# beecave-homelab/VibeVoice-ROCm

Measured on AMD Instinct MI355X. Metric: audio-sec/s, higher is better.
Workload: dtype bf16

## Files before the change

### vibevoice_rocm_amd/csrc/vv_common.h

```cpp
#ifndef VV_COMMON_H
#define VV_COMMON_H
#include <hip/hip_runtime.h>
#include <stdarg.h>
#include <stdint.h>
#include "vv_hip.h"

int vv_set_error(int code, const char* fmt, ...);

#define VV_CHECK_LAUNCH(name)                                                                    \
  do {                                                                                           \
    hipError_t e_ = hipGetLastError();                                                           \
    if (e_ != hipSuccess) return vv_set_error(VV_E_HIP, "%s: %s", name, hipGetErrorString(e_));  \
  } while (0)

#define VV_TRY(expr)            \
  do {                          \
    int rc_ = (expr);           \
    if (rc_) return rc_;        \
  } while (0)

int vv_launch_gemv_stream(const vv_lin_args& a, hipStream_t s);
int vv_launch_gemv_rows(const vv_lin_args& a, float* part, size_t part_floats, int* tickets, size_t n_tickets, hipStream_t s);
size_t vv_gemv_rows_part_floats(int n, int dual);
size_t vv_gemv_rows_tickets(int n);
int vv_gemv_rows_init();
void vv_gemv_rows_set(int on, int blocks, int pers);
int vv_linear_ws(const vv_lin_args* a, const void* f1, const void* f2, float* part, size_t part_floats, int* tickets, size_t n_tickets,
                 vv_stream_t stream, const vv_w8* q1 = nullptr, const vv_w8* q2 = nullptr);
int vv_launch_mfma_gemm(const vv_lin_args& a, hipStream_t s);
int vv_mfma_gemm_init();
int vv_launch_attn_decode(const float* qkv, int64_t ld_qkv, int R, int heads, const vv_kv* kv, int layer, const float2* rope, const int* lens, float* out,
                          int64_t ldo, float* part, int* tickets, int nsplit, int part_cap, hipStream_t s);
int vv_attn_decode_ws(const float* qkv, int64_t ld_qkv, int R, int heads, const vv_kv* kv, int layer, const float* rope_table, const int* lens, float* out,
                      int64_t ldo, float* part, int* tickets, int nsplit, int part_cap, vv_stream_t stream);
int vv_launch_attn_prefill(const float* qkv, int64_t ld_qkv, int R, int heads, const vv_kv* kv, int layer, const int* lens, const int* cache_rows,
                           float* out, int64_t ldo, hipStream_t s);
int vv_head_init_fused(const vv_head* h, const float* noise, float* Xs, float* Ms, float* h0, int64_t ldh, hipStream_t s);
bool vv_head_boundary_supported(const vv_head* h);
int vv_head_boundary_fused(const vv_head* h, const float* hrows, int64_t ldh, const float* shift, const float* scale, int64_t ld_mod, float cfg,
                           const vv_dpm_coef* k, float* Xs, float* Ms, float* h_out, int64_t ldh_out, float* latent_out, hipStream_t s);
int vv_head_boundary_batch(const vv_head* h, const float* hrows, int64_t ldh, const float* shift, const float* scale, int64_t ld_mod, float cfg,
                           const vv_dpm_coef* k, float* Xs, float* Ms, int64_t state_stride, float* h_out, int64_t ldh_out, float* latent_out,
                           int64_t latent_stride, int B, hipStream_t s,
                           const float* nx = nullptr, int64_t nx_stride = 0);
int vv_head_sde_proj_fused(const vv_head* h, const float* sde_noise, int64_t ld_sde, int n_steps, int B, float* NX, hipStream_t s);
int vv_fused_init();
int vv_head_pre_fused(const vv_head* h, const float* cond2, int64_t ld_cond, const float* temb, int n_steps, void* c_bf16, const float* noise,
                      float* Xs, float* Ms, float* h0, int64_t ldh, hipStream_t s);
int vv_launch_connector_pair(const vv_connector* ac, const vv_connector* sem, const float* latent, const float* semfeat, float* out, int64_t ldo, int rows_out,
                             float* ws, hipStream_t s);
int vv_head_modulations_fused(const vv_head* h, const void* c_bf16, int rows, float* const* mod, float* modf, hipStream_t s);
struct vv_conv_ctx_item { float* pad; float* state; int ctx, T, C; const float* dw_w; float* hs; int affine; float scale, bias; };
int vv_conv_ctx_batch(const vv_conv_ctx_item* items, int n, int scatter, hipStream_t s);
int vv_block1d_init();
int vv_launch_block1d(const vv_block& B, int wdt, const float* x, float* out, int T, int C, float eps, hipStream_t s);
void vv_block1d_set_fused(int on);
void vv_block1d_set_blocks(int b);
int vv_convffn_init();
int vv_launch_convffn(const vv_block& B, int wdt, const float* x, float* y, void* hidden, float* hist_new, float* out, int T, int C, float eps,
                      hipStream_t s);
void vv_convffn_set(int on);
int vv_launch_ffn_in_row(const vv_block& B, int wdt, const float* x, float* y, float* hidden, float* hist_new, int C, float eps, hipStream_t s);
void vv_convffn_set_t1(int on);
int vv_launch_ffn_in_row_hs(const vv_block& B, int wdt, const float* x, float* y, float* hidden, float* hist_new, int C, float eps, hipStream_t s);
void vv_convffn_set_t1hs(int on);
void vv_convffn_set_rows(int c, int rows);
void vv_convffn_set_c128(int on);
bool vv_convffn_prefers(int wdt, int T, int C);
int vv_launch_skinny(const vv_lin_args& a, hipStream_t s);
void vv_skinny_set(int on, int min_m, int max_m);
int vv_rmsnorm_rows(const float* x, int64_t ldx, const float* w, float eps, int rows, int n, float* out, int64_t ldo, hipStream_t s);

#ifdef __HIPCC__
__device__ __forceinline__ float vv_gelu_as(float v) {
  const float x = v * 0.70710678118654752440f, ax = fabsf(x);
  const float t = __builtin_amdgcn_rcpf(fmaf(0.3275911f, ax, 1.0f));
  const float poly = t * fmaf(t, fmaf(t, fmaf(t, fmaf(t, 1.061405429f, -1.453152027f), 1.421413741f), -0.284496736f), 0.254829592f);
  const float erf_abs = 1.0f - poly * __expf(-ax * ax);
  return 0.5f * v * (1.0f + copysignf(erf_abs, x));
}

__device__ __forceinline__ float vv_wave_sum(float v) {
#define VV_DPP_ADD(ctrl) v += __int_as_float(__builtin_amdgcn_update_dpp(0, __float_as_int(v), ctrl, 0xF, 0xF, true))
  VV_DPP_ADD(0xB1);
  VV_DPP_ADD(0x4E);
  VV_DPP_ADD(0x141);
  VV_DPP_ADD(0x140);
#undef VV_DPP_ADD
  const float r0 = __int_as_float(__builtin_amdgcn_readlane(__float_as_int(v), 0));
  const float r1 = __int_as_float(__builtin_amdgcn_readlane(__float_as_int(v), 16));
  const float r2 = __int_as_float(__builtin_amdgcn_readlane(__float_as_int(v), 32));
  const float r3 = __int_as_float(__builtin_amdgcn_readlane(__float_as_int(v), 48));
  return (r0 + r1) + (r2 + r3);
}
#endif

#endif
```

### vibevoice_rocm_amd/csrc/vv_convffn.hip

```cpp
#include <hip/hip_runtime.h>
#include <hip/hip_bf16.h>
#include <stdint.h>

#include "vv_hip.h"
#include "vv_common.h"

namespace {

typedef unsigned short bf16_t;
typedef __bf16 bf16x8 __attribute__((ext_vector_type(8)));
typedef float f32x16 __attribute__((ext_vector_type(16)));
typedef float f32x4 __attribute__((ext_vector_type(4)));
typedef unsigned int u32x4 __attribute__((ext_vector_type(4)));

#ifdef VV_CF_TIMING
__device__ unsigned long long g_cf_t[8];
#define CSTAMP(i) do { if (blockIdx.x == 0 && blockIdx.y == 0 && threadIdx.x == 0) { const long long t_ = wall_clock64(); g_cf_t[i] += (unsigned long long)(t_ - tprev_); tprev_ = t_; } } while (0)
#else
#define CSTAMP(i) do { } while (0)
#endif

constexpr int TR2 = 16;
constexpr int HALO = 6;

__device__ __forceinline__ unsigned int pack2(float a, float b) {
  const __hip_bfloat16 x = __float2bfloat16(a), y = __float2bfloat16(b);
  return (unsigned int)(*reinterpret_cast<const bf16_t*>(&x)) | ((unsigned int)(*reinterpret_cast<const bf16_t*>(&y)) << 16);
}
__device__ __forceinline__ float sq4(const float4 v) { return v.x * v.x + v.y * v.y + v.z * v.z + v.w * v.w; }

template <int C, int TRV, int NT = 256> struct InLay {
  static constexpr int VW = C >= 256 ? 4 : 2;
  static constexpr int F4 = C / 4;
  static constexpr int FV = C / VW;
  static constexpr int TPR = FV < NT ? FV : NT;
  static constexpr int NWV = NT / 64;
  static constexpr int CPT = FV / TPR;
  static constexpr int RP = NT / TPR;
  static constexpr int NI = (TRV + HALO + RP - 1) / RP;
  static constexpr int WR = NI * RP;
  static constexpr int WPR = TPR / 64;
  static constexpr int P1 = C + 8;
  static constexpr int ST = C / (16 * NWV);
  static constexpr size_t XN = (size_t)WR * C * 4;
  static constexpr size_t RED = (size_t)NWV * 16 * 64 * 4;
  static constexpr size_t XH = (size_t)(WR - HALO) * P1 * 2;
  static constexpr size_t PART = (size_t)2 * WR * 8 * 4;
  static constexpr size_t LDS = (XN > RED ? XN : RED) + XH + PART;
};

template <int VW> __device__ __forceinline__ void ldv(const float* p, float (&o)[VW]) {
  if constexpr (VW == 4) { const float4 t = *reinterpret_cast<const float4*>(p); o[0] = t.x; o[1] = t.y; o[2] = t.z; o[3] = t.w; }
  else { const float2 t = *reinterpret_cast<const float2*>(p); o[0] = t.x; o[1] = t.y; }
}
template <int VW> __device__ __forceinline__ void stv(float* p, const float (&o)[VW]) {
  if constexpr (VW == 4) *reinterpret_cast<float4*>(p) = make_float4(o[0], o[1], o[2], o[3]);
  else *reinterpret_cast<float2*>(p) = make_float2(o[0], o[1]);
}

template <int C, int TRV, bool HF32, int NT>
__global__ __launch_bounds__(NT) void ffn_in_kernel(const float* __restrict__ x, float* __restrict__ y, void* __restrict__ hidden_v,
                                                     float* __restrict__ hist_new, int T, const vv_block B, float eps) {
  using L = InLay<C, TRV, NT>;
  constexpr int TR = TRV, CPT = L::CPT, VW = L::VW, NWV = L::NWV;
#ifdef VV_CF_TIMING
  long long tprev_ = wall_clock64();
#endif
  extern __shared__ __attribute__((aligned(16))) unsigned char smem[];
  float* xn = reinterpret_cast<float*>(smem);
  float* red = reinterpret_cast<float*>(smem);
  bf16_t* xh = reinterpret_cast<bf16_t*>(smem + (L::XN > L::RED ? L::XN : L::RED));
  float* part = reinterpret_cast<float*>(smem + (L::XN > L::RED ? L::XN : L::RED) + L::XH);
  float* part2 = part + L::WR * 8;
  const int tid = threadIdx.x, lane = tid & 63, wave = __builtin_amdgcn_readfirstlane(tid >> 6);
  const int n0 = blockIdx.x * 32;
  const int t0 = blockIdx.y * TR;
  const int rows = min(TR, T - t0);
  const int lm = lane & 31, hk = (lane >> 5) * 8;

  const int rloc = wave / L::WPR, slot = wave % L::WPR;
  int c0[CPT];
#pragma unroll
  for (int j = 0; j < CPT; ++j) c0[j] = VW * (tid % L::TPR + L::TPR * j);
  const float* hb = B.hist ? B.hist : x;
  const float hkeep = B.hist ? 1.f : 0.f;
  float own[L::NI][CPT][VW];
#pragma unroll
  for (int i = 0; i < L::NI; ++i) {
    const int w = rloc + L::RP * i, t = t0 - HALO + w;
    const bool isx = t >= 0;
    const float* src = isx ? x + (int64_t)min(t, T - 1) * C : hb + (int64_t)(B.hist ? HALO + t : 0) * C;
    const float keep = (w < rows + HALO) ? (isx ? 1.f : hkeep) : 0.f;
#pragma unroll
    for (int j = 0; j < CPT; ++j) {
      ldv<VW>(src + c0[j], own[i][j]);
#pragma unroll
      for (int e = 0; e < VW; ++e) own[i][j][e] *= keep;
    }
  }
  float nw[CPT][VW], db[CPT][VW], gm[CPT][VW], fw[CPT][VW];
  float tap[CPT][VW * 7];
#pragma unroll
  for (int j = 0; j < CPT; ++j) {
    ldv<VW>(B.norm_w + c0[j], nw[j]);
    ldv<VW>(B.dw_b + c0[j], db[j]);
    ldv<VW>(B.gamma + c0[j], gm[j]);
    ldv<VW>(B.ffn_norm_w + c0[j], fw[j]);
#pragma unroll
    for (int q = 0; q < 7; ++q) {
      float tq[VW];
      ldv<VW>(B.dw_w + (size_t)c0[j] * 7 + VW * q, tq);
#pragma unroll
      for (int e = 0; e < VW; ++e) tap[j][VW * q + e] = tq[e];
    }
  }
  u32x4 wf[L::ST];
  {
    const bf16_t* wr = reinterpret_cast<const bf16_t*>(B.w1) + (int64_t)(n0 + lm) * C + wave * (C / NWV) + hk;
#pragma unroll
    for (int s = 0; s < L::ST; ++s) wf[s] = *reinterpret_cast<const u32x4*>(wr + s * 16);
  }
  const int eg = wave & 3;
  const float4 b1v = *reinterpret_cast<const float4*>(B.b1 + n0 + 8 * eg + 4 * (lane >> 5));
  __builtin_amdgcn_sched_barrier(0);

  CSTAMP(0);
#pragma unroll
  for (int i = 0; i < L::NI; ++i) {
    const int w = rloc + L::RP * i;
    float q = 0.f;
#pragma unroll
    for (int j = 0; j < CPT; ++j)
#pragma unroll
      for (int e = 0; e < VW; ++e) q = fmaf(own[i][j][e], own[i][j][e], q);
    const float s = vv_wave_sum(q);
    if (lane == 0) part[w * 8 + slot] = s;
  }
  __syncthreads();
  CSTAMP(1);
#pragma unroll
  for (int i = 0; i < L::NI; ++i) {
    const int w = rloc + L::RP * i, t = t0 - HALO + w;
    float ss = part[w * 8];
#pragma unroll
    for (int sl = 1; sl < L::WPR; ++sl) ss += part[w * 8 + sl];
    const bool isx = t >= 0;
    const float rstd = isx ? rsqrtf(ss / (float)C + eps) : 1.f;
#pragma unroll
    for (int j = 0; j < CPT; ++j) {
      float o[VW];
#pragma unroll
      for (int e = 0; e < VW; ++e) o[e] = own[i][j][e] * rstd * (isx ? nw[j][e] : 1.f);
      stv<VW>(xn + w * C + c0[j], o);
    }
  }
  __syncthreads();
  CSTAMP(2);

  float y1[L::NI][CPT][VW];
#pragma unroll
  for (int i = 0; i < L::NI; ++i) {
#pragma unroll
    for (int j = 0; j < CPT; ++j)
#pragma unroll
      for (int e = 0; e < VW; ++e) y1[i][j][e] = 0.f;
    if (L::RP * i + L::RP - 1 < HALO) continue;
    const int w = rloc + L::RP * i, tt = w - HALO;
    const int tc = max(tt, 0);
    const float ok = (tt >= 0 && tt < rows) ? 1.f : 0.f;
    float q = 0.f;
#pragma unroll
    for (int j = 0; j < CPT; ++j) {
      float s[VW];
#pragma unroll
      for (int e = 0; e < VW; ++e) s[e] = db[j][e];
#pragma unroll
      for (int k = 0; k < 7; ++k) {
        float v[VW];
        ldv<VW>(xn + (tc + k) * C + c0[j], v);
#pragma unroll
        for (int e = 0; e < VW; ++e) s[e] = fmaf(tap[j][7 * e + k], v[e], s[e]);
      }
#pragma unroll
      for (int e = 0; e < VW; ++e) {
        y1[i][j][e] = (own[i][j][e] + gm[j][e] * s[e]) * ok;
        q = fmaf(y1[i][j][e], y1[i][j][e], q);
      }
    }
    const float s2 = vv_wave_sum(q);
    if (lane == 0) part2[w * 8 + slot] = s2;
  }
  if (hist_new && blockIdx.x == 0 && t0 + TR >= T) {
    for (int e = tid; e < HALO * L::F4; e += NT) {
      const int j = e / L::F4, c4 = e - j * L::F4;
      *reinterpret_cast<float4*>(hist_new + (size_t)j * C + 4 * c4) = *reinterpret_cast<const float4*>(xn + (size_t)(T - t0 + j) * C + 4 * c4);
    }
  }
  __syncthreads();
  CSTAMP(3);
  {
    const int ys0 = blockIdx.x * (C / (int)gridDim.x);
#pragma unroll
    for (int i = 0; i < L::NI; ++i) {
      if (L::RP * i + L::RP - 1 < HALO) continue;
      const int w = rloc + L::RP * i, tt = w - HALO;
      if (tt >= 0) {
        float ss = part2[w * 8];
#pragma unroll
        for (int sl = 1; sl < L::WPR; ++sl) ss += part2[w * 8 + sl];
        const float rstd = rsqrtf(ss / (float)C + eps);
#pragma unroll
        for (int j = 0; j < CPT; ++j) {
          if constexpr (VW == 4) {
            uint2 p;
            p.x = pack2(y1[i][j][0] * rstd * fw[j][0], y1[i][j][1] * rstd * fw[j][1]);
            p.y = pack2(y1[i][j][2] * rstd * fw[j][2], y1[i][j][3] * rstd * fw[j][3]);
            *reinterpret_cast<uint2*>(xh + tt * L::P1 + c0[j]) = p;
          } else {
            *reinterpret_cast<unsigned int*>(xh + tt * L::P1 + c0[j]) = pack2(y1[i][j][0] * rstd * fw[j][0], y1[i][j][1] * rstd * fw[j][1]);
          }
          const bool mine = c0[j] >= ys0 && c0[j] < ys0 + C / (int)gridDim.x;
          if (mine && tt < rows) stv<VW>(y + (int64_t)(t0 + tt) * C + c0[j], y1[i][j]);
        }
      }
    }
  }
  __syncthreads();

  CSTAMP(4);
  f32x16 acc;
#pragma unroll
  for (int i = 0; i < 16; ++i) acc[i] = 0.f;
  {
    const bf16_t* xf = xh + min(lm, TR - 1) * L::P1 + wave * (C / NWV) + hk;
#pragma unroll
    for (int s = 0; s < L::ST; ++s) {
      const u32x4 xb = *reinterpret_cast<const u32x4*>(xf + s * 16);
      acc = __builtin_amdgcn_mfma_f32_32x32x16_bf16(__builtin_bit_cast(bf16x8, wf[s]), __builtin_bit_cast(bf16x8, xb), acc, 0, 0, 0);
    }
  }
#pragma unroll
  for (int r = 0; r < 16; ++r) red[(wave * 16 + r) * 64 + lane] = acc[r];
  __syncthreads();
  CSTAMP(5);
  {
    const int m = lane & 31;
    if (m < rows && wave < 4) {
      float v[4];
#pragma unroll
      for (int i = 0; i < 4; ++i) {
        float s = 0.f;
#pragma unroll
        for (int w4 = 0; w4 < NWV; ++w4) s += red[(w4 * 16 + 4 * eg + i) * 64 + lane];
        v[i] = s;
      }
      const float g0 = vv_gelu_as(v[0] + b1v.x), g1 = vv_gelu_as(v[1] + b1v.y), g2 = vv_gelu_as(v[2] + b1v.z), g3 = vv_gelu_as(v[3] + b1v.w);
      const int64_t ho = (int64_t)(t0 + m) * (4 * C) + n0 + 8 * eg + 4 * (lane >> 5);
      if (HF32) {
        *reinterpret_cast<float4*>(reinterpret_cast<float*>(hidden_v) + ho) = make_float4(g0, g1, g2, g3);
      } else {
        uint2 p;
        p.x = pack2(g0, g1);
        p.y = pack2(g2, g3);
        *reinterpret_cast<uint2*>(reinterpret_cast<bf16_t*>(hidden_v) + ho) = p;
      }
    }
  }
  CSTAMP(6);
}


__global__ __launch_bounds__(256) void ffn_in_row_kernel(const float* __restrict__ x, float* __restrict__ y, float* __restrict__ hidden,
                                                         float* __restrict__ hist_new, const vv_block B, float eps) {
  constexpr int C = 2048, P1 = C + 8, ST = C / 64;
  __shared__ __attribute__((aligned(16))) bf16_t xh[P1];
  __shared__ float red[4 * 16 * 64];
  __shared__ float part[8];
  const int tid = threadIdx.x, lane = tid & 63, wave = __builtin_amdgcn_readfirstlane(tid >> 6);
  const int n0 = blockIdx.x * 32;
  const int lm = lane & 31, hk = (lane >> 5) * 8;
  float xv[2][4], hsv[2][4], dl[2][4], nw[2][4], db[2][4], gm[2][4], fw[2][4];
  int c0[2];
#pragma unroll
  for (int j = 0; j < 2; ++j) {
    c0[j] = 4 * (tid + 256 * j);
    ldv<4>(x + c0[j], xv[j]);
    ldv<4>(B.norm_w + c0[j], nw[j]);
    ldv<4>(B.hs + c0[j], hsv[j]);
    ldv<4>(B.dw_last + c0[j], dl[j]);
    ldv<4>(B.dw_b + c0[j], db[j]);
    ldv<4>(B.gamma + c0[j], gm[j]);
    ldv<4>(B.ffn_norm_w + c0[j], fw[j]);
  }
  const bool keeper = hist_new && blockIdx.x == 0;
  float hrow[5][2][4];
  if (keeper) {
#pragma unroll
    for (int r = 0; r < 5; ++r)
#pragma unroll
      for (int j = 0; j < 2; ++j) ldv<4>(B.hist + (size_t)(r + 1) * C + c0[j], hrow[r][j]);
  }
  u32x4 wf[ST];
  {
    const bf16_t* wr = reinterpret_cast<const bf16_t*>(B.w1) + (int64_t)(n0 + lm) * C + wave * (C / 4) + hk;
#pragma unroll
    for (int s = 0; s < ST; ++s) wf[s] = *reinterpret_cast<const u32x4*>(wr + s * 16);
  }
  const int eg = wave;
  const float4 b1v = *reinterpret_cast<const float4*>(B.b1 + n0 + 8 * eg + 4 * (lane >> 5));
  __builtin_amdgcn_sched_barrier(0);
  float q = 0.f;
#pragma unroll
  for (int j = 0; j < 2; ++j)
#pragma unroll
    for (int e = 0; e < 4; ++e) q = fmaf(xv[j][e], xv[j][e], q);
  q = vv_wave_sum(q);
  if (lane == 0) part[wave] = q;
  __syncthreads();
  const float rstd1 = rsqrtf(((part[0] + part[1]) + (part[2] + part[3])) / (float)C + eps);
  float yv[2][4], xn[2][4];
  float q2 = 0.f;
#pragma unroll
  for (int j = 0; j < 2; ++j)
#pragma unroll
    for (int e = 0; e < 4; ++e) {
      xn[j][e] = xv[j][e] * rstd1 * nw[j][e];
      const float sc = db[j][e] + hsv[j][e] + dl[j][e] * xn[j][e];
      yv[j][e] = xv[j][e] + gm[j][e] * sc;
      q2 = fmaf(yv[j][e], yv[j][e], q2);
    }
  q2 = vv_wave_sum(q2);
  if (lane == 0) part[4 + wave] = q2;
  if (keeper) {
#pragma unroll
    for (int j = 0; j < 2; ++j) {
#pragma unroll
      for (int r = 0; r < 5; ++r) stv<4>(hist_new + (size_t)r * C + c0[j], hrow[r][j]);
      stv<4>(hist_new + (size_t)5 * C + c0[j], xn[j]);
    }
  }
  __syncthreads();
  const float rstd2 = rsqrtf(((part[4] + part[5]) + (part[6] + part[7])) / (float)C + eps);
  {
    const int ys0 = blockIdx.x * (C / (int)gridDim.x);
#pragma unroll
    for (int j = 0; j < 2; ++j) {
      uint2 p;
      p.x = pack2(yv[j][0] * rstd2 * fw[j][0], yv[j][1] * rstd2 * fw[j][1]);
      p.y = pack2(yv[j][2] * rstd2 * fw[j][2], yv[j][3] * rstd2 * fw[j][3]);
      *reinterpret_cast<uint2*>(xh + c0[j]) = p;
      if (c0[j] >= ys0 && c0[j] < ys0 + C / (int)gridDim.x) stv<4>(y + c0[j], yv[j]);
    }
  }
  __syncthreads();
  f32x16 acc;
#pragma unroll
  for (int i = 0; i < 16; ++i) acc[i] = 0.f;
  {
    const bf16_t* xf = xh + wave * (C / 4) + hk;
#pragma unroll
    for (int s = 0; s < ST; ++s) {
      const u32x4 xb = *reinterpret_cast<const u32x4*>(xf + s * 16);
      acc = __builtin_amdgcn_mfma_f32_32x32x16_bf16(__builtin_bit_cast(bf16x8, wf[s]), __builtin_bit_cast(bf16x8, xb), acc, 0, 0, 0);
    }
  }
#pragma unroll
  for (int r = 0; r < 16; ++r) red[(wave * 16 + r) * 64 + lane] = acc[r];
  __syncthreads();
  if ((lane & 31) == 0) {
    float v[4];
#pragma unroll
    for (int i = 0; i < 4; ++i) {
      float s = 0.f;
#pragma unroll
      for (int w4 = 0; w4 < 4; ++w4) s += red[(w4 * 16 + 4 * eg + i) * 64 + lane];
      v[i] = s;
    }
    *reinterpret_cast<float4*>(hidden + n0 + 8 * eg + 4 * (lane >> 5)) =
        make_float4(vv_gelu_as(v[0] + b1v.x), vv_gelu_as(v[1] + b1v.y), vv_gelu_as(v[2] + b1v.z), vv_gelu_as(v[3] + b1v.w));
  }
}

template <int C, int NW>
__global__ __launch_bounds__(64 * NW) void ffn_out_kernel(const bf16_t* __restrict__ hidden, const float* res, float* out, const float* __restrict__ hist_new,
                                                          int T, const vv_block B) {
  constexpr int K = 4 * C, KW = K / NW, ST = KW / 32;
  __shared__ float red[NW * 4 * 64];
  const int tid = threadIdx.x, lane = tid & 63, wave = tid >> 6;
  const int n0 = blockIdx.x * 16, t0 = blockIdx.y * TR2;
  const int r16 = lane & 15, kq = lane >> 4;
  u32x4 wf[ST], hf[ST];
  {
    const bf16_t* wr = reinterpret_cast<const bf16_t*>(B.w2) + (int64_t)(n0 + r16) * K + wave * KW + 8 * kq;
    const bf16_t* hr = hidden + (int64_t)min(t0 + r16, T - 1) * K + wave * KW + 8 * kq;
#pragma unroll
    for (int s = 0; s < ST; ++s) {
      wf[s] = *reinterpret_cast<const u32x4*>(wr + s * 32);
      hf[s] = *reinterpret_cast<const u32x4*>(hr + s * 32);
    }
  }
  const int ei = (tid >> 6) & 3, el = tid & 63;
  const int en = n0 + 4 * (el >> 4) + ei, em = t0 + (el & 15);
  const bool ev = em < T && tid < 256;
  const float b2v = B.b2[en], fgv = B.ffn_gamma[en];
  const float rv = ev ? res[(int64_t)em * C + en] : 0.f;
  const bool mover = hist_new && B.hist && blockIdx.x == 0 && blockIdx.y == 0;
  constexpr int HN = (HALO * C / 4 + 64 * NW - 1) / (64 * NW);
  float4 hv[HN];
  if (mover) {
#pragma unroll
    for (int i = 0; i < HN; ++i) {
      const int e = tid + 64 * NW * i;
      hv[i] = e < HALO * C / 4 ? *reinterpret_cast<const float4*>(hist_new + 4 * (size_t)e) : make_float4(0.f, 0.f, 0.f, 0.f);
    }
  }
  f32x4 acc = {0.f, 0.f, 0.f, 0.f};
#pragma unroll
  for (int s = 0; s < ST; ++s)
    acc = __builtin_amdgcn_mfma_f32_16x16x32_bf16(__builtin_bit_cast(bf16x8, wf[s]), __builtin_bit_cast(bf16x8, hf[s]), acc, 0, 0, 0);
#pragma unroll
  for (int i = 0; i < 4; ++i) red[(wave * 4 + i) * 64 + lane] = acc[i];
  __syncthreads();
  if (ev) {
    float s = 0.f;
#pragma unroll
    for (int w4 = 0; w4 < NW; ++w4) s += red[(w4 * 4 + ei) * 64 + el];
    out[(int64_t)em * C + en] = rv + fgv * (s + b2v);
  }
  if (mover) {
#pragma unroll
    for (int i = 0; i < HN; ++i) {
      const int e = tid + 64 * NW * i;
      if (e < HALO * C / 4) *reinterpret_cast<float4*>(B.hist + 4 * (size_t)e) = hv[i];
    }
  }
}

template <int NST, int NB>
__global__ __launch_bounds__(256) void skinny_kernel(const float* __restrict__ x, int64_t ldx, int M, const bf16_t* __restrict__ W, int K,
                                                     const float* __restrict__ bias, float* __restrict__ out, int64_t ldo) {
  __shared__ float red[4 * 4 * 64];
  const int tid = threadIdx.x, lane = tid & 63, wave = tid >> 6;
  const int n0 = blockIdx.x * 16, t0 = blockIdx.y * 16;
  const int r16 = lane & 15, kq = lane >> 4;
  const int kb = wave * (32 * NST * NB) + 8 * kq;
  const bf16_t* wr = W + (int64_t)(n0 + r16) * K + kb;
  const float* xr = x + (int64_t)min(t0 + r16, M - 1) * ldx + kb;
  const int ei = tid >> 6, el = tid & 63;
  const int en = n0 + 4 * (el >> 4) + ei, em = t0 + (el & 15);
  const float bv = bias ? bias[en] : 0.f;
  f32x4 acc = {0.f, 0.f, 0.f, 0.f};
#pragma unroll
  for (int b = 0; b < NB; ++b) {
    u32x4 wf[NST];
    float4 xa[NST], xb[NST];
#pragma unroll
    for (int s = 0; s < NST; ++s) {
      wf[s] = *reinterpret_cast<const u32x4*>(wr + 32 * (b * NST + s));
      xa[s] = *reinterpret_cast<const float4*>(xr + 32 * (b * NST + s));
      xb[s] = *reinterpret_cast<const float4*>(xr + 32 * (b * NST + s) + 4);
    }
#pragma unroll
    for (int s = 0; s < NST; ++s) {
      u32x4 p;
      p.x = pack2(xa[s].x, xa[s].y); p.y = pack2(xa[s].z, xa[s].w); p.z = pack2(xb[s].x, xb[s].y); p.w = pack2(xb[s].z, xb[s].w);
      acc = __builtin_amdgcn_mfma_f32_16x16x32_bf16(__builtin_bit_cast(bf16x8, wf[s]), __builtin_bit_cast(bf16x8, p), acc, 0, 0, 0);
    }
  }
#pragma unroll
  for (int i = 0; i < 4; ++i) red[(wave * 4 + i) * 64 + lane] = acc[i];
  __syncthreads();
  if (em < M) {
    float v = 0.f;
#pragma unroll
    for (int w4 = 0; w4 < 4; ++w4) v += red[(w4 * 4 + ei) * 64 + el];
    out[(int64_t)em * ldo + en] = v + bv;
  }
}

int g_skinny = 1, g_skinny_min_m = 5, g_skinny_max_m = 2048;

int g_on = 1;

template <int C> constexpr int in_threads() { return (C == 512 || C == 1024) ? 512 : 256; }

template <int C, int TRV, int NW>
int launch_c(const vv_block& B, const float* x, float* y, void* hidden, float* hist_new, float* out, int T, float eps, hipStream_t s) {
  float* hn = B.hist ? hist_new : nullptr;
  constexpr int NT = in_threads<C>();
  constexpr size_t lds = InLay<C, TRV, NT>::LDS;
  hipLaunchKernelGGL((ffn_in_kernel<C, TRV, false, NT>), dim3(4 * C / 32, (T + TRV - 1) / TRV), dim3(NT), lds, s, x, y, hidden, hn, T, B, eps);
  hipLaunchKernelGGL((ffn_out_kernel<C, NW>), dim3(C / 16, (T + TR2 - 1) / TR2), dim3(64 * NW), 0, s, reinterpret_cast<const bf16_t*>(hidden), y, out, hn, T, B);
  return hipGetLastError() == hipSuccess ? 1 : vv_set_error(VV_E_HIP, "vv_convffn: launch failed");
}

int g_trv512 = 8, g_trv256 = 16, g_trv128 = 32;
int g_c128 = 1;

}

#ifdef VV_CF_TIMING
extern "C" int vv_convffn_debug_times(unsigned long long* out8, int reset) {
  if (hipMemcpyFromSymbol(out8, HIP_SYMBOL(g_cf_t), 8 * sizeof(unsigned long long)) != hipSuccess) return -1;
  if (reset) { unsigned long long z[8] = {0}; if (hipMemcpyToSymbol(HIP_SYMBOL(g_cf_t), z, sizeof(z)) != hipSuccess) return -1; }
  return 0;
}
#endif
void vv_convffn_set(int on) { g_on = on; }
void vv_convffn_set_rows(int c, int rows) { if (c == 512) g_trv512 = rows; else if (c == 256) g_trv256 = rows; else if (c == 128) g_trv128 = rows; }
void vv_convffn_set_c128(int on) { g_c128 = on; }
bool vv_convffn_prefers(int wdt, int T, int C) { return g_on && g_c128 && wdt == VV_BF16 && C == 128 && T >= 3 && T <= 1024; }
void vv_skinny_set(int on, int min_m, int max_m) { g_skinny = on; if (min_m > 0) g_skinny_min_m = min_m; if (max_m > 0) g_skinny_max_m = max_m; }

int vv_launch_skinny(const vv_lin_args& a, hipStream_t s) {
  if (!g_skinny || a.wdt != VV_BF16 || a.w2 || a.pro != VV_PRO_NONE || a.act != VV_ACT_NONE || a.gate || a.res || a.mod_scale || a.flags) return 0;
  if (a.m < g_skinny_min_m || a.m > g_skinny_max_m || a.n % 16 || a.ldx % 4 || a.ldx == 0 || ((uintptr_t)a.x % 16) || ((uintptr_t)a.w % 16)) return 0;
  dim3 grid(a.n / 16, (a.m + 15) / 16);
  const bf16_t* W = reinterpret_cast<const bf16_t*>(a.w);
#define VV_SK(NSTV, NBV) hipLaunchKernelGGL((skinny_kernel<NSTV, NBV>), grid, dim3(256), 0, s, a.x, a.ldx, a.m, W, a.k, a.bias, a.out, a.ldo)
  switch (a.k) {
    case 128: VV_SK(1, 1); break;
    case 256: VV_SK(2, 1); break;
    case 512: VV_SK(4, 1); break;
    case 1024: VV_SK(8, 1); break;
    case 2048: VV_SK(16, 1); break;
    case 2560: VV_SK(20, 1); break;
    case 5120: VV_SK(20, 2); break;
    default: return 0;
  }
#undef VV_SK
  return 1;
}

int vv_convffn_init() {
#define VV_CF_ATTR(CC, TT)                                                                                                                  \
  { constexpr int nt_ = in_threads<CC>(); constexpr int l_ = (int)InLay<CC, TT, nt_>::LDS;                                                 \
    if (hipFuncSetAttribute(reinterpret_cast<const void*>(&ffn_in_kernel<CC, TT, false, nt_>), hipFuncAttributeMaxDynamicSharedMemorySize, l_) != hipSuccess) \
      return vv_set_error(VV_E_HIP, "vv_convffn_init: cannot raise the LDS limit"); }
  VV_CF_ATTR(128, 16) VV_CF_ATTR(128, 32) VV_CF_ATTR(256, 8) VV_CF_ATTR(256, 16) VV_CF_ATTR(256, 32) VV_CF_ATTR(512, 8) VV_CF_ATTR(512, 16) VV_CF_ATTR(512, 32) VV_CF_ATTR(1024, 8)
#undef VV_CF_ATTR
  {
    constexpr int l1 = (int)InLay<2048, 1, 256>::LDS;
    if (hipFuncSetAttribute(reinterpret_cast<const void*>(&ffn_in_kernel<2048, 1, true, 256>), hipFuncAttributeMaxDynamicSharedMemorySize, l1) != hipSuccess)
      return vv_set_error(VV_E_HIP, "vv_convffn_init: cannot raise the LDS limit");
  }
  return 0;
}

int g_t1 = 1;
void vv_convffn_set_t1(int on) { g_t1 = on; }

int vv_launch_ffn_in_row(const vv_block& B, int wdt, const float* x, float* y, float* hidden, float* hist_new, int C, float eps, hipStream_t s) {
  if (!g_on || !g_t1 || wdt != VV_BF16 || C != 2048 || !B.hist) return 0;
  auto a16 = [](const void* q) { return q && ((uintptr_t)q % 16) == 0; };
  if (!a16(B.w1) || !a16(B.b1) || !a16(B.gamma) || !a16(B.norm_w) || !a16(B.ffn_norm_w) || !a16(B.dw_b) || !a16(B.dw_w) || !a16(x) || !a16(y) ||
      !a16(hidden) || !a16(hist_new) || !a16(B.hist) || x == y)
    return 0;
  constexpr size_t lds = InLay<2048, 1, 256>::LDS;
  hipLaunchKernelGGL((ffn_in_kernel<2048, 1, true, 256>), dim3(4 * 2048 / 32, 1), dim3(256), lds, s, x, y, hidden, hist_new, 1, B, eps);
  return hipGetLastError() == hipSuccess ? 1 : vv_set_error(VV_E_HIP, "vv_convffn: launch failed");
}

int g_t1hs = 1;
void vv_convffn_set_t1hs(int on) { g_t1hs = on; }

int vv_launch_ffn_in_row_hs(const vv_block& B, int wdt, const float* x, float* y, float* hidden, float* hist_new, int C, float eps, hipStream_t s) {
  if (!g_on || !g_t1 || !g_t1hs || wdt != VV_BF16 || C != 2048 || !B.hist || !B.hs || !B.dw_last) return 0;
  auto a16 = [](const void* q) { return q && ((uintptr_t)q % 16) == 0; };
  if (!a16(B.w1) || !a16(B.b1) || !a16(B.gamma) || !a16(B.norm_w) || !a16(B.ffn_norm_w) || !a16(B.dw_b) || !a16(B.dw_last) || !a16(B.hs) || !a16(x) ||
      !a16(y) || !a16(hidden) || !a16(hist_new) || !a16(B.hist) || x == y)
    return 0;
  hipLaunchKernelGGL(ffn_in_row_kernel, dim3(4 * 2048 / 32), dim3(256), 0, s, x, y, hidden, hist_new, B, eps);
  return hipGetLastError() == hipSuccess ? 1 : vv_set_error(VV_E_HIP, "vv_convffn: launch failed");
}

int vv_launch_convffn(const vv_block& B, int wdt, const float* x, float* y, void* hidden, float* hist_new, float* out, int T, int C, float eps,
                      hipStream_t s) {
  if (!g_on || wdt != VV_BF16 || T < 3 || (C != 128 && C != 256 && C != 512 && C != 1024) || (C == 1024 && T > 64)) return 0;
  if (C == 128 ? (!g_c128 || T > 1024) : T > 256) return 0;
  auto a16 = [](const void* q) { return q && ((uintptr_t)q % 16) == 0; };
  if (!a16(B.w1) || !a16(B.w2) || !a16(B.b1) || !B.b2 || !a16(B.gamma) || !B.ffn_gamma || !a16(B.norm_w) || !a16(B.ffn_norm_w) || !a16(B.dw_b) ||
      !a16(B.dw_w) || !a16(x) || !a16(y) || !a16(hidden) || !a16(hist_new) || !out || (B.hist && !a16(B.hist)))
    return 0;
  {
    const uintptr_t xa = (uintptr_t)x, ya = (uintptr_t)y, bytes = (uintptr_t)T * C * 4;
    if (xa < ya + bytes && ya < xa + bytes) return 0;
  }
  if (C == 128) {
    if (g_trv128 == 16) return launch_c<128, 16, 4>(B, x, y, hidden, hist_new, out, T, eps, s);
    return launch_c<128, 32, 4>(B, x, y, hidden, hist_new, out, T, eps, s);
  }
  if (C == 256) {
    if (g_trv256 == 8) return launch_c<256, 8, 4>(B, x, y, hidden, hist_new, out, T, eps, s);
    if (g_trv256 == 16) return launch_c<256, 16, 4>(B, x, y, hidden, hist_new, out, T, eps, s);
    return launch_c<256, 32, 4>(B, x, y, hidden, hist_new, out, T, eps, s);
  }
  if (C == 512) {
    if (g_trv512 == 8) return launch_c<512, 8, 4>(B, x, y, hidden, hist_new, out, T, eps, s);
    if (g_trv512 == 16) return launch_c<512, 16, 4>(B, x, y, hidden, hist_new, out, T, eps, s);
    return launch_c<512, 32, 4>(B, x, y, hidden, hist_new, out, T, eps, s);
  }
  return launch_c<1024, 8, 8>(B, x, y, hidden, hist_new, out, T, eps, s);
}

extern "C" size_t vv_block_mid_ws_bytes(int T, int C) { return (size_t)T * C * 4 + (size_t)T * 4 * C * 2 + (size_t)HALO * C * 4 + 64; }

extern "C" int vv_block_mid(const vv_block* b, int wdt, const float* x, float* out, void* ws, int T, int C, float eps, vv_stream_t stream) {
  if (!b || !x || !out || !ws || T <= 0) return vv_set_error(VV_E_ARG, "vv_block_mid: bad args");
  float* y = reinterpret_cast<float*>(ws);
  char* hidden = reinterpret_cast<char*>(ws) + (size_t)T * C * 4;
  float* hn = reinterpret_cast<float*>(hidden + (size_t)T * 4 * C * 2);
  const int rc = vv_launch_convffn(*b, wdt, x, y, hidden, hn, out, T, C, eps, (hipStream_t)stream);
  if (rc < 0) return rc;
  if (rc == 0) return vv_set_error(VV_E_UNSUPPORTED, "vv_block_mid: shape not covered (C=%d T=%d wdt=%d)", C, T, wdt);
  return 0;
}
```

### vibevoice_rocm_amd/csrc/vv_kernels.hip

```cpp
#include <hip/hip_runtime.h>
#include <hip/hip_bf16.h>
#include <stdint.h>
#include <stdio.h>
#include <string.h>
#include <math.h>

#include "vv_hip.h"
#include "vv_common.h"

static thread_local char g_err[512] = "";

int vv_set_error(int code, const char* fmt, ...) {
  va_list ap;
  va_start(ap, fmt);
  vsnprintf(g_err, sizeof(g_err), fmt, ap);
  va_end(ap);
  return code;
}

extern "C" const char* vv_last_error(void) { return g_err; }
extern "C" int vv_abi_version(void) { return 6; }
int vv_mixer_init();
extern "C" int vv_init(void) {
  VV_TRY(vv_mixer_init());
  VV_TRY(vv_mfma_gemm_init());
  VV_TRY(vv_block1d_init());
  VV_TRY(vv_convffn_init());
  VV_TRY(vv_gemv_rows_init());
  return vv_fused_init();
}
static float* g_rows_part = nullptr;
static int* g_rows_tk = nullptr;
static const size_t G_ROWS_PART_FLOATS = (size_t)4 << 20, G_ROWS_TICKETS = 4096;
static int rows_scratch(int on) {
  if (on && !g_rows_part) {
    if (hipMalloc(&g_rows_part, G_ROWS_PART_FLOATS * sizeof(float)) != hipSuccess || hipMalloc(&g_rows_tk, G_ROWS_TICKETS * sizeof(int)) != hipSuccess ||
        hipMemset(g_rows_tk, 0, G_ROWS_TICKETS * sizeof(int)) != hipSuccess)
      return vv_set_error(VV_E_HIP, "vv_tune: gemv_rows_scratch allocation failed");
  }
  if (!on && g_rows_part) { (void)hipFree(g_rows_part); (void)hipFree(g_rows_tk); g_rows_part = nullptr; g_rows_tk = nullptr; }
  return 0;
}
void vv_gemv_rows_set_dbg(int d);
void vv_gemv_rows_set_atomic(int on);
void vv_gemv_stream_set_blocks(int b);
void vv_gemv_stream_set_waves(int w);
void vv_gemv_stream_set_opt(int o);
void vv_gemv_stream_set_long(int cap, int ku);
void vv_gemv_stream_set_dual_rw(int r);
void vv_gemv_stream_set_small_rw(int r);
void vv_mfma_set_mt(int mt);
void vv_mfma_set_tiled_rows(int r);
void vv_mfma_set_tiled_bk128(int on);
void vv_mfma_set_tiled_small(int t);
void vv_mfma_set_tiled_dual_bk64(int on);
void vv_mfma_set_tiled_small_dual(int t);
void vv_mfma_set_tiled_small_k(int k);
void vv_mixer_set_rows(int on);
void vv_mfma_set_mt_prefill(int mt);
extern int g_attn_group;
void vv_attn_decode_set_gqa(int on);
void vv_attn_decode_set_gqa_keys(int k);
extern "C" int vv_tune(const char* key, int value) {
  if (key && !strcmp(key, "gemv_long_cap")) { vv_gemv_stream_set_long(value, 0); return 0; }
  if (key && !strcmp(key, "gemv_long_ku")) { vv_gemv_stream_set_long(0, value); return 0; }
  if (key && !strcmp(key, "gemv_blocks")) { vv_gemv_stream_set_blocks(value); return 0; }
  if (key && !strcmp(key, "gemv_waves")) { vv_gemv_stream_set_waves(value); return 0; }
  if (key && !strcmp(key, "gemv_rows")) { vv_gemv_rows_set(value, 0, -1); return 0; }
  if (key && !strcmp(key, "gemv_rows_blocks")) { vv_gemv_rows_set(-1, value, -1); return 0; }
  if (key && !strcmp(key, "gemv_rows_pers")) { vv_gemv_rows_set(-1, 0, value); return 0; }
  if (key && !strcmp(key, "gemv_rows_scratch")) return rows_scratch(value);
  if (key && !strcmp(key, "gemv_rows_dbg")) { vv_gemv_rows_set_dbg(value); return 0; }
  if (key && !strcmp(key, "gemv_rows_atomic")) { vv_gemv_rows_set_atomic(value); return 0; }
  if (key && !strcmp(key, "gemv_opt")) { vv_gemv_stream_set_opt(value); return 0; }
  if (key && !strcmp(key, "gemv_dual_rw")) { vv_gemv_stream_set_dual_rw(value); return 0; }
  if (key && !strcmp(key, "gemv_small_rw")) { vv_gemv_stream_set_small_rw(value); return 0; }
  if (key && !strcmp(key, "mixer_rows")) { vv_mixer_set_rows(value); return 0; }
  if (key && !strcmp(key, "block1d_fused")) { vv_block1d_set_fused(value); return 0; }
  if (key && !strcmp(key, "block1d_blocks")) { vv_block1d_set_blocks(value); return 0; }
  if (key && !strcmp(key, "convffn")) { vv_convffn_set(value); return 0; }
  if (key && !strcmp(key, "convffn_t1")) { vv_convffn_set_t1(value); return 0; }
  if (key && !strcmp(key, "convffn_t1hs")) { vv_convffn_set_t1hs(value); return 0; }
  if (key && !strcmp(key, "convffn_rows512")) { vv_convffn_set_rows(512, value); return 0; }
  if (key && !strcmp(key, "convffn_rows256")) { vv_convffn_set_rows(256, value); return 0; }
  if (key && !strcmp(key, "convffn_rows128")) { vv_convffn_set_rows(128, value); return 0; }
  if (key && !strcmp(key, "convffn_c128")) { vv_convffn_set_c128(value); return 0; }
  if (key && !strcmp(key, "skinny")) { vv_skinny_set(value, 0, 0); return 0; }
  if (key && !strcmp(key, "skinny_min_m")) { vv_skinny_set(1, value, 0); return 0; }
  if (key && !strcmp(key, "skinny_max_m")) { vv_skinny_set(1, 0, value); return 0; }
  if (key && !strcmp(key, "mfma_tiled_bk128")) { vv_mfma_set_tiled_bk128(value); return 0; }
  if (key && !strcmp(key, "attn_group")) { g_attn_group = value; return 0; }
  if (key && !strcmp(key, "attn_gqa")) { vv_attn_decode_set_gqa(value); return 0; }
  if (key && !strcmp(key, "attn_gqa_keys")) { vv_attn_decode_set_gqa_keys(value); return 0; }
  if (key && !strcmp(key, "mfma_tiled_small_k")) { vv_mfma_set_tiled_small_k(value); return 0; }
  if (key && !strcmp(key, "mfma_tiled_dual_bk64")) { vv_mfma_set_tiled_dual_bk64(value); return 0; }
  if (key && !strcmp(key, "mfma_tiled_small_dual")) { vv_mfma_set_tiled_small_dual(value); return 0; }
  if (key && !strcmp(key, "mfma_tiled_small")) { vv_mfma_set_tiled_small(value); return 0; }
  if (key && !strcmp(key, "mfma_tiled_rows")) { vv_mfma_set_tiled_rows(value); return 0; }
  if (key && !strcmp(key, "mfma_mt")) { vv_mfma_set_mt(value); return 0; }
  if (key && !strcmp(key, "mfma_mt_prefill")) { vv_mfma_set_mt_prefill(value); return 0; }
  return vv_set_error(VV_E_ARG, "vv_tune: unknown key");
}

typedef unsigned short bf16_t;

__device__ __forceinline__ float bf2f(unsigned int u16) { return __uint_as_float(u16 << 16); }
__device__ __forceinline__ float wave_sum(float v) {
#pragma unroll
  for (int o = 32; o > 0; o >>= 1) v += __shfl_xor(v, o);
  return v;
}
__device__ __forceinline__ float wave_sum_dpp(float v) { return vv_wave_sum(v); }
__device__ __forceinline__ float silu_f(float v) { return v / (1.0f + expf(-v)); }
__device__ __forceinline__ float gelu_f(float v) { return 0.5f * v * (1.0f + erff(v * 0.70710678118654752440f)); }

template <typename WT> struct WL;
template <> struct WL<float> {
  static __device__ __forceinline__ void load8(const float* p, float (&o)[8]) {
    const float4 a = *reinterpret_cast<const float4*>(p);
    const float4 b = *reinterpret_cast<const float4*>(p + 4);
    o[0] = a.x; o[1] = a.y; o[2] = a.z; o[3] = a.w; o[4] = b.x; o[5] = b.y; o[6] = b.z; o[7] = b.w;
  }
  static __device__ __forceinline__ void load4(const float* p, float (&o)[4]) {
    const float4 a = *reinterpret_cast<const float4*>(p);
    o[0] = a.x; o[1] = a.y; o[2] = a.z; o[3] = a.w;
  }
  static __device__ __forceinline__ float load1(const float* p) { return *p; }
};
template <> struct WL<bf16_t> {
  static __device__ __forceinline__ void load8(const bf16_t* p, float (&o)[8]) {
    const uint4 v = *reinterpret_cast<const uint4*>(p);
    o[0] = __uint_as_float(v.x << 16); o[1] = __uint_as_float(v.x & 0xffff0000u);
    o[2] = __uint_as_float(v.y << 16); o[3] = __uint_as_float(v.y & 0xffff0000u);
    o[4] = __uint_as_float(v.z << 16); o[5] = __uint_as_float(v.z & 0xffff0000u);
    o[6] = __uint_as_float(v.w << 16); o[7] = __uint_as_float(v.w & 0xffff0000u);
  }
  static __device__ __forceinline__ void load4(const bf16_t* p, float (&o)[4]) {
    const uint2 v = *reinterpret_cast<const uint2*>(p);
    o[0] = __uint_as_float(v.x << 16); o[1] = __uint_as_float(v.x & 0xffff0000u);
    o[2] = __uint_as_float(v.y << 16); o[3] = __uint_as_float(v.y & 0xffff0000u);
  }
  static __device__ __forceinline__ float load1(const bf16_t* p) { return bf2f(*p); }
};

__device__ __forceinline__ void lin_epilogue(const vv_lin_args& a, int m, int n, float v, float v2) {
  if (a.bias) v += a.bias[n];
  if (a.act == VV_ACT_GELU) v = gelu_f(v);
  else if (a.act == VV_ACT_SWIGLU) v = silu_f(v) * v2;
  if (a.gate) v *= a.gate_ld ? a.gate[(int64_t)m * a.gate_ld + n] : a.gate[n];
  if (a.res) v += a.res[(int64_t)m * a.ldres + n];
  a.out[(int64_t)m * a.ldo + n] = v;
}

#define GEMV_THREADS 256

template <int M>
__device__ __forceinline__ void row_stats(const vv_lin_args& a, float* red, float (&rstd)[M]) {
  const int tid = threadIdx.x, lane = tid & 63, wave = tid >> 6;
  float ss[M];
#pragma unroll
  for (int m = 0; m < M; ++m) {
    const float* xr = a.x + (int64_t)m * a.ldx;
    float s = 0.f;
    for (int k = tid; k < a.k; k += GEMV_THREADS) { const float v = xr[k]; s += v * v; }
    ss[m] = wave_sum(s);
  }
  if (lane == 0) {
#pragma unroll
    for (int m = 0; m < M; ++m) red[wave * M + m] = ss[m];
  }
  __syncthreads();
#pragma unroll
  for (int m = 0; m < M; ++m) {
    const float t = red[m] + red[M + m] + red[2 * M + m] + red[3 * M + m];
    rstd[m] = rsqrtf(t / (float)a.k + a.eps);
  }
  __syncthreads();
}

template <int M>
__device__ __forceinline__ void stage_chunk(const vv_lin_args& a, float* xs, int kc0, int kc, int kcp, const float (&rstd)[M]) {
  for (int idx = threadIdx.x; idx < M * kcp; idx += GEMV_THREADS) {
    const int m = idx / kcp, kk = idx - m * kcp;
    float v = 0.f;
    if (kk < kc) {
      const int k = kc0 + kk;
      v = a.x[(int64_t)m * a.ldx + k];
      if (a.pro == VV_PRO_RMSNORM) {
        v *= rstd[m];
        if (a.norm_w) v *= a.norm_w[k];
        if (a.mod_scale) v = v * (1.0f + a.mod_scale[(int64_t)m * a.ld_mod + k]) + a.mod_shift[(int64_t)m * a.ld_mod + k];
      } else if (a.pro == VV_PRO_SILU) {
        v = silu_f(v);
      }
    }
    xs[idx] = v;
  }
}

template <typename WT, int M, bool DUAL, int KSPLIT, int RW>
__global__ __launch_bounds__(GEMV_THREADS) void gemv_kernel(const vv_lin_args a, const int KC) {
  extern __shared__ __attribute__((aligned(16))) float smem[];
  float* red = smem;
  float* xs = smem + 64 * 4;
  const int tid = threadIdx.x, lane = tid & 63, wave = tid >> 6;
  const int K = a.k, N = a.n;
  const WT* __restrict__ W = reinterpret_cast<const WT*>(a.w);
  const WT* __restrict__ W2 = reinterpret_cast<const WT*>(a.w2);

  float rstd[M];
#pragma unroll
  for (int m = 0; m < M; ++m) rstd[m] = 1.f;
  if (a.pro == VV_PRO_RMSNORM) row_stats<M>(a, red, rstd);

  const int row0 = (KSPLIT == 1 ? (blockIdx.x * 4 + wave) : blockIdx.x) * RW;
  float acc[RW][M], acc2[DUAL ? RW : 1][M];
#pragma unroll
  for (int r = 0; r < RW; ++r)
#pragma unroll
    for (int m = 0; m < M; ++m) { acc[r][m] = 0.f; if (DUAL) acc2[r][m] = 0.f; }

  for (int kc0 = 0; kc0 < K; kc0 += KC) {
    const int kc = min(KC, K - kc0);
    const int kcp = (kc + 7) & ~7;
    if (kc0 > 0) __syncthreads();
    stage_chunk<M>(a, xs, kc0, kc, kcp, rstd);
    __syncthreads();
    const int kstart = (KSPLIT == 1 ? lane : (wave * 64 + lane)) * 8;
    const int kstep = (KSPLIT == 1 ? 64 : 256) * 8;
#pragma unroll 2
    for (int k = kstart; k < kc; k += kstep) {
      float w[RW][8], w2[DUAL ? RW : 1][8];
#pragma unroll
      for (int r = 0; r < RW; ++r) {
        const int n = min(row0 + r, N - 1);
        WL<WT>::load8(W + (int64_t)n * K + kc0 + k, w[r]);
        if (DUAL) WL<WT>::load8(W2 + (int64_t)n * K + kc0 + k, w2[r]);
      }
#pragma unroll
// ... 1461 lines not shown
```

Before: 38.47.

## Process multiple 32-column output blocks per ffn_in workgroup with prefetched weights

Each ffn_in workgroup now handles NB consecutive 32-wide output column blocks, reusing the normalized/conv input tile and its register copy of the x fragments across blocks. Weight fragments for the next blocks are prefetched into a rotating register set, and the reduction buffer is double-buffered so consecutive blocks can overlap. Defaults set NB=2 for C=128/256/512, and the C=128 row tile drops from 32 to 16. The aim is to amortize the per-workgroup prologue (load, norm, conv) over more output columns, at the cost of fewer workgroups, more registers and extra LDS.

After: 38.63, median of 6. About the same (+0.4%).

```diff
diff --git a/vibevoice_rocm_amd/csrc/vv_common.h b/vibevoice_rocm_amd/csrc/vv_common.h
--- a/vibevoice_rocm_amd/csrc/vv_common.h
+++ b/vibevoice_rocm_amd/csrc/vv_common.h
@@ -66,6 +66,7 @@
 void vv_convffn_set_t1hs(int on);
 void vv_convffn_set_rows(int c, int rows);
 void vv_convffn_set_c128(int on);
+void vv_convffn_set_blocks(int c, int nb);
 bool vv_convffn_prefers(int wdt, int T, int C);
 int vv_launch_skinny(const vv_lin_args& a, hipStream_t s);
 void vv_skinny_set(int on, int min_m, int max_m);
diff --git a/vibevoice_rocm_amd/csrc/vv_convffn.hip b/vibevoice_rocm_amd/csrc/vv_convffn.hip
--- a/vibevoice_rocm_amd/csrc/vv_convffn.hip
+++ b/vibevoice_rocm_amd/csrc/vv_convffn.hip
@@ -29,7 +29,7 @@
 }
 __device__ __forceinline__ float sq4(const float4 v) { return v.x * v.x + v.y * v.y + v.z * v.z + v.w * v.w; }
 
-template <int C, int TRV, int NT = 256> struct InLay {
+template <int C, int TRV, int NT = 256, int NB = 1> struct InLay {
   static constexpr int VW = C >= 256 ? 4 : 2;
   static constexpr int F4 = C / 4;
   static constexpr int FV = C / VW;
@@ -43,7 +43,7 @@
   static constexpr int P1 = C + 8;
   static constexpr int ST = C / (16 * NWV);
   static constexpr size_t XN = (size_t)WR * C * 4;
-  static constexpr size_t RED = (size_t)NWV * 16 * 64 * 4;
+  static constexpr size_t RED = (size_t)(NB > 1 ? 2 : 1) * NWV * 16 * 64 * 4;
   static constexpr size_t XH = (size_t)(WR - HALO) * P1 * 2;
   static constexpr size_t PART = (size_t)2 * WR * 8 * 4;
   static constexpr size_t LDS = (XN > RED ? XN : RED) + XH + PART;
@@ -58,10 +58,10 @@
   else *reinterpret_cast<float2*>(p) = make_float2(o[0], o[1]);
 }
 
-template <int C, int TRV, bool HF32, int NT>
+template <int C, int TRV, bool HF32, int NT, int NB = 1>
 __global__ __launch_bounds__(NT) void ffn_in_kernel(const float* __restrict__ x, float* __restrict__ y, void* __restrict__ hidden_v,
                                                      float* __restrict__ hist_new, int T, const vv_block B, float eps) {
-  using L = InLay<C, TRV, NT>;
+  using L = InLay<C, TRV, NT, NB>;
   constexpr int TR = TRV, CPT = L::CPT, VW = L::VW, NWV = L::NWV;
 #ifdef VV_CF_TIMING
   long long tprev_ = wall_clock64();
@@ -73,7 +73,7 @@
   float* part = reinterpret_cast<float*>(smem + (L::XN > L::RED ? L::XN : L::RED) + L::XH);
   float* part2 = part + L::WR * 8;
   const int tid = threadIdx.x, lane = tid & 63, wave = __builtin_amdgcn_readfirstlane(tid >> 6);
-  const int n0 = blockIdx.x * 32;
+  const int n0 = blockIdx.x * 32 * NB;
   const int t0 = blockIdx.y * TR;
   const int rows = min(TR, T - t0);
   const int lm = lane & 31, hk = (lane >> 5) * 8;
@@ -114,14 +114,17 @@
       for (int e = 0; e < VW; ++e) tap[j][VW * q + e] = tq[e];
     }
   }
-  u32x4 wf[L::ST];
-  {
-    const bf16_t* wr = reinterpret_cast<const bf16_t*>(B.w1) + (int64_t)(n0 + lm) * C + wave * (C / NWV) + hk;
-#pragma unroll
-    for (int s = 0; s < L::ST; ++s) wf[s] = *reinterpret_cast<const u32x4*>(wr + s * 16);
-  }
+  constexpr int NS = NB < 3 ? NB : 3;
+  u32x4 wf[NS][L::ST];
+  const bf16_t* wr = reinterpret_cast<const bf16_t*>(B.w1) + (int64_t)(n0 + lm) * C + wave * (C / NWV) + hk;
+#pragma unroll
+  for (int b = 0; b < (NB < 2 ? NB : 2); ++b)
+#pragma unroll
+    for (int s = 0; s < L::ST; ++s) wf[b][s] = *reinterpret_cast<const u32x4*>(wr + (int64_t)32 * b * C + s * 16);
   const int eg = wave & 3;
-  const float4 b1v = *reinterpret_cast<const float4*>(B.b1 + n0 + 8 * eg + 4 * (lane >> 5));
+  float4 b1v[NB];
+#pragma unroll
+  for (int b = 0; b < NB; ++b) b1v[b] = *reinterpret_cast<const float4*>(B.b1 + n0 + 32 * b + 8 * eg + 4 * (lane >> 5));
   __builtin_amdgcn_sched_barrier(0);
 
   CSTAMP(0);
@@ -228,22 +231,33 @@
   __syncthreads();
 
   CSTAMP(4);
-  f32x16 acc;
-#pragma unroll
-  for (int i = 0; i < 16; ++i) acc[i] = 0.f;
-  {
-    const bf16_t* xf = xh + min(lm, TR - 1) * L::P1 + wave * (C / NWV) + hk;
+  const bf16_t* xf = xh + min(lm, TR - 1) * L::P1 + wave * (C / NWV) + hk;
+  u32x4 xb[NB > 1 ? L::ST : 1];
+  if constexpr (NB > 1) {
+#pragma unroll
+    for (int s = 0; s < L::ST; ++s) xb[s] = *reinterpret_cast<const u32x4*>(xf + s * 16);
+  }
+#pragma unroll
+  for (int b = 0; b < NB; ++b) {
+    if (b + 2 < NB) {
+#pragma unroll
+      for (int s = 0; s < L::ST; ++s) wf[(b + 2) % NS][s] = *reinterpret_cast<const u32x4*>(wr + (int64_t)32 * (b + 2) * C + s * 16);
+    }
+    f32x16 acc;
+#pragma unroll
+    for (int i = 0; i < 16; ++i) acc[i] = 0.f;
 #pragma unroll
     for (int s = 0; s < L::ST; ++s) {
-      const u32x4 xb = *reinterpret_cast<const u32x4*>(xf + s * 16);
-      acc = __builtin_amdgcn_mfma_f32_32x32x16_bf16(__builtin_bit_cast(bf16x8, wf[s]), __builtin_bit_cast(bf16x8, xb), acc, 0, 0, 0);
-    }
-  }
-#pragma unroll
-  for (int r = 0; r < 16; ++r) red[(wave * 16 + r) * 64 + lane] = acc[r];
-  __syncthreads();
-  CSTAMP(5);
-  {
+      u32x4 xv;
+      if constexpr (NB > 1) xv = xb[s];
+      else xv = *reinterpret_cast<const u32x4*>(xf + s * 16);
+      acc = __builtin_amdgcn_mfma_f32_32x32x16_bf16(__builtin_bit_cast(bf16x8, wf[b % NS][s]), __builtin_bit_cast(bf16x8, xv), acc, 0, 0, 0);
+    }
+    float* rb = red + (NB > 1 ? (b & 1) : 0) * (NWV * 16 * 64);
+#pragma unroll
+    for (int r = 0; r < 16; ++r) rb[(wave * 16 + r) * 64 + lane] = acc[r];
+    __syncthreads();
+    CSTAMP(5);
     const int m = lane & 31;
     if (m < rows && wave < 4) {
       float v[4];
@@ -251,11 +265,11 @@
       for (int i = 0; i < 4; ++i) {
         float s = 0.f;
 #pragma unroll
-        for (int w4 = 0; w4 < NWV; ++w4) s += red[(w4 * 16 + 4 * eg + i) * 64 + lane];
+        for (int w4 = 0; w4 < NWV; ++w4) s += rb[(w4 * 16 + 4 * eg + i) * 64 + lane];
         v[i] = s;
       }
-      const float g0 = vv_gelu_as(v[0] + b1v.x), g1 = vv_gelu_as(v[1] + b1v.y), g2 = vv_gelu_as(v[2] + b1v.z), g3 = vv_gelu_as(v[3] + b1v.w);
-      const int64_t ho = (int64_t)(t0 + m) * (4 * C) + n0 + 8 * eg + 4 * (lane >> 5);
+      const float g0 = vv_gelu_as(v[0] + b1v[b].x), g1 = vv_gelu_as(v[1] + b1v[b].y), g2 = vv_gelu_as(v[2] + b1v[b].z), g3 = vv_gelu_as(v[3] + b1v[b].w);
+      const int64_t ho = (int64_t)(t0 + m) * (4 * C) + n0 + 32 * b + 8 * eg + 4 * (lane >> 5);
       if (HF32) {
         *reinterpret_cast<float4*>(reinterpret_cast<float*>(hidden_v) + ho) = make_float4(g0, g1, g2, g3);
       } else {
@@ -265,8 +279,8 @@
         *reinterpret_cast<uint2*>(reinterpret_cast<bf16_t*>(hidden_v) + ho) = p;
       }
     }
-  }
-  CSTAMP(6);
+    CSTAMP(6);
+  }
 }
 
 
@@ -484,17 +498,18 @@
 
 template <int C> constexpr int in_threads() { return (C == 512 || C == 1024) ? 512 : 256; }
 
-template <int C, int TRV, int NW>
+template <int C, int TRV, int NW, int NB = 1>
 int launch_c(const vv_block& B, const float* x, float* y, void* hidden, float* hist_new, float* out, int T, float eps, hipStream_t s) {
   float* hn = B.hist ? hist_new : nullptr;
   constexpr int NT = in_threads<C>();
-  constexpr size_t lds = InLay<C, TRV, NT>::LDS;
-  hipLaunchKernelGGL((ffn_in_kernel<C, TRV, false, NT>), dim3(4 * C / 32, (T + TRV - 1) / TRV), dim3(NT), lds, s, x, y, hidden, hn, T, B, eps);
+  constexpr size_t lds = InLay<C, TRV, NT, NB>::LDS;
+  hipLaunchKernelGGL((ffn_in_kernel<C, TRV, false, NT, NB>), dim3(4 * C / (32 * NB), (T + TRV - 1) / TRV), dim3(NT), lds, s, x, y, hidden, hn, T, B, eps);
   hipLaunchKernelGGL((ffn_out_kernel<C, NW>), dim3(C / 16, (T + TR2 - 1) / TR2), dim3(64 * NW), 0, s, reinterpret_cast<const bf16_t*>(hidden), y, out, hn, T, B);
   return hipGetLastError() == hipSuccess ? 1 : vv_set_error(VV_E_HIP, "vv_convffn: launch failed");
 }
 
-int g_trv512 = 8, g_trv256 = 16, g_trv128 = 32;
+int g_trv512 = 8, g_trv256 = 16, g_trv128 = 16;
+int g_nb1024 = 1, g_nb512 = 2, g_nb256 = 2, g_nb128 = 2;
 int g_c128 = 1;
 
 }
@@ -509,6 +524,10 @@
 void vv_convffn_set(int on) { g_on = on; }
 void vv_convffn_set_rows(int c, int rows) { if (c == 512) g_trv512 = rows; else if (c == 256) g_trv256 = rows; else if (c == 128) g_trv128 = rows; }
 void vv_convffn_set_c128(int on) { g_c128 = on; }
+void vv_convffn_set_blocks(int c, int nb) {
+  if (nb != 1 && nb != 2 && nb != 4) return;
+  if (c == 1024) g_nb1024 = nb; else if (c == 512) g_nb512 = nb; else if (c == 256) g_nb256 = nb; else if (c == 128) g_nb128 = nb;
+}
 bool vv_convffn_prefers(int wdt, int T, int C) { return g_on && g_c128 && wdt == VV_BF16 && C == 128 && T >= 3 && T <= 1024; }
 void vv_skinny_set(int on, int min_m, int max_m) { g_skinny = on; if (min_m > 0) g_skinny_min_m = min_m; if (max_m > 0) g_skinny_max_m = max_m; }
 
@@ -533,12 +552,14 @@
 }
 
 int vv_convffn_init() {
-#define VV_CF_ATTR(CC, TT)                                                                                                                  \
-  { constexpr int nt_ = in_threads<CC>(); constexpr int l_ = (int)InLay<CC, TT, nt_>::LDS;                                                 \
-    if (hipFuncSetAttribute(reinterpret_cast<const void*>(&ffn_in_kernel<CC, TT, false, nt_>), hipFuncAttributeMaxDynamicSharedMemorySize, l_) != hipSuccess) \
+#define VV_CF_ATTR_NB(CC, TT, NBV)                                                                                                          \
+  { constexpr int nt_ = in_threads<CC>(); constexpr int l_ = (int)InLay<CC, TT, nt_, NBV>::LDS;                                            \
+    if (hipFuncSetAttribute(reinterpret_cast<const void*>(&ffn_in_kernel<CC, TT, false, nt_, NBV>), hipFuncAttributeMaxDynamicSharedMemorySize, l_) != hipSuccess) \
       return vv_set_error(VV_E_HIP, "vv_convffn_init: cannot raise the LDS limit"); }
+#define VV_CF_ATTR(CC, TT) VV_CF_ATTR_NB(CC, TT, 1) VV_CF_ATTR_NB(CC, TT, 2) VV_CF_ATTR_NB(CC, TT, 4)
   VV_CF_ATTR(128, 16) VV_CF_ATTR(128, 32) VV_CF_ATTR(256, 8) VV_CF_ATTR(256, 16) VV_CF_ATTR(256, 32) VV_CF_ATTR(512, 8) VV_CF_ATTR(512, 16) VV_CF_ATTR(512, 32) VV_CF_ATTR(1024, 8)
 #undef VV_CF_ATTR
+#undef VV_CF_ATTR_NB
   {
     constexpr int l1 = (int)InLay<2048, 1, 256>::LDS;
     if (hipFuncSetAttribute(reinterpret_cast<const void*>(&ffn_in_kernel<2048, 1, true, 256>), hipFuncAttributeMaxDynamicSharedMemorySize, l1) != hipSuccess)
@@ -586,21 +607,25 @@
     const uintptr_t xa = (uintptr_t)x, ya = (uintptr_t)y, bytes = (uintptr_t)T * C * 4;
     if (xa < ya + bytes && ya < xa + bytes) return 0;
   }
+#define VV_CF_NB(CC, TT, NWV, NBV)                                                                                                          \
+  (NBV == 4 ? launch_c<CC, TT, NWV, 4>(B, x, y, hidden, hist_new, out, T, eps, s)                                                         \
+            : NBV == 2 ? launch_c<CC, TT, NWV, 2>(B, x, y, hidden, hist_new, out, T, eps, s) : launch_c<CC, TT, NWV, 1>(B, x, y, hidden, hist_new, out, T, eps, s))
   if (C == 128) {
-    if (g_trv128 == 16) return launch_c<128, 16, 4>(B, x, y, hidden, hist_new, out, T, eps, s);
-    return launch_c<128, 32, 4>(B, x, y, hidden, hist_new, out, T, eps, s);
+    if (g_trv128 == 16) return VV_CF_NB(128, 16, 4, g_nb128);
+    return VV_CF_NB(128, 32, 4, g_nb128);
   }
   if (C == 256) {
-    if (g_trv256 == 8) return launch_c<256, 8, 4>(B, x, y, hidden, hist_new, out, T, eps, s);
-    if (g_trv256 == 16) return launch_c<256, 16, 4>(B, x, y, hidden, hist_new, out, T, eps, s);
-    return launch_c<256, 32, 4>(B, x, y, hidden, hist_new, out, T, eps, s);
+    if (g_trv256 == 8) return VV_CF_NB(256, 8, 4, g_nb256);
+    if (g_trv256 == 16) return VV_CF_NB(256, 16, 4, g_nb256);
+    return VV_CF_NB(256, 32, 4, g_nb256);
   }
   if (C == 512) {
-    if (g_trv512 == 8) return launch_c<512, 8, 4>(B, x, y, hidden, hist_new, out, T, eps, s);
-    if (g_trv512 == 16) return launch_c<512, 16, 4>(B, x, y, hidden, hist_new, out, T, eps, s);
-    return launch_c<512, 32, 4>(B, x, y, hidden, hist_new, out, T, eps, s);
-  }
-  return launch_c<1024, 8, 8>(B, x, y, hidden, hist_new, out, T, eps, s);
+    if (g_trv512 == 8) return VV_CF_NB(512, 8, 4, g_nb512);
+    if (g_trv512 == 16) return VV_CF_NB(512, 16, 4, g_nb512);
+    return VV_CF_NB(512, 32, 4, g_nb512);
+  }
+  return VV_CF_NB(1024, 8, 8, g_nb1024);
+#undef VV_CF_NB
 }
 
 extern "C" size_t vv_block_mid_ws_bytes(int T, int C) { return (size_t)T * C * 4 + (size_t)T * 4 * C * 2 + (size_t)HALO * C * 4 + 64; }
diff --git a/vibevoice_rocm_amd/csrc/vv_kernels.hip b/vibevoice_rocm_amd/csrc/vv_kernels.hip
--- a/vibevoice_rocm_amd/csrc/vv_kernels.hip
+++ b/vibevoice_rocm_amd/csrc/vv_kernels.hip
@@ -85,6 +85,10 @@
   if (key && !strcmp(key, "convffn_rows256")) { vv_convffn_set_rows(256, value); return 0; }
   if (key && !strcmp(key, "convffn_rows128")) { vv_convffn_set_rows(128, value); return 0; }
   if (key && !strcmp(key, "convffn_c128")) { vv_convffn_set_c128(value); return 0; }
+  if (key && !strcmp(key, "convffn_nb1024")) { vv_convffn_set_blocks(1024, value); return 0; }
+  if (key && !strcmp(key, "convffn_nb512")) { vv_convffn_set_blocks(512, value); return 0; }
+  if (key && !strcmp(key, "convffn_nb256")) { vv_convffn_set_blocks(256, value); return 0; }
+  if (key && !strcmp(key, "convffn_nb128")) { vv_convffn_set_blocks(128, value); return 0; }
   if (key && !strcmp(key, "skinny")) { vv_skinny_set(value, 0, 0); return 0; }
   if (key && !strcmp(key, "skinny_min_m")) { vv_skinny_set(1, value, 0); return 0; }
   if (key && !strcmp(key, "skinny_max_m")) { vv_skinny_set(1, 0, value); return 0; }
```
